# bitsauce/Carla-ppo

Measured on NVIDIA H100. Metric: VAE frames/sec @ batch 4096, higher is better.
Workload: dtype f32

## Files before the change

carla_ppo_b200/csrc/tc_tapgemm.cu:

```cuda
#include "tapgemm.cuh"
#include "tc_common.cuh"

namespace cpb {

namespace {

using namespace tc;

template <int BN, int PASSES>
struct TcCfg {
    static constexpr int B_TILE_BYTES = BN * TBK * 4;
    static constexpr int B_IMAGES = PASSES == 3 ? 2 : 1;
    static constexpr int STAGE_BYTES = A_TILE_BYTES + B_IMAGES * B_TILE_BYTES;
    static constexpr int STAGES = 200 * 1024 / STAGE_BYTES;
    static constexpr int SMEM_BYTES = STAGES * STAGE_BYTES + 1024;
};
constexpr int CHUNK_KB = 4;

constexpr int kConsumerWarps = 8;
constexpr int kLoaderWarp0 = 8;
constexpr int kLoaderWarps = 4;
constexpr int kLoaderThreads = kLoaderWarps * 32;
constexpr int kTcThreads = 384;

int g_tc_cluster = 1;
int g_tc_clusters[2][2] = {{0, 0}, {0, 0}};

__device__ __forceinline__ uint32_t cluster_ctarank() { uint32_t r; asm volatile("mov.u32 %0, %%cluster_ctarank;" : "=r"(r)); return r; }
__device__ __forceinline__ uint32_t cluster_id_x() { uint32_t r; asm volatile("mov.u32 %0, %%clusterid.x;" : "=r"(r)); return r; }
__device__ __forceinline__ uint32_t cluster_count_x() { uint32_t r; asm volatile("mov.u32 %0, %%nclusterid.x;" : "=r"(r)); return r; }
__device__ __forceinline__ void cluster_sync_all() {
    asm volatile("barrier.cluster.arrive.release.aligned;" ::: "memory");
    asm volatile("barrier.cluster.wait.acquire.aligned;" ::: "memory");
}
__device__ __forceinline__ void mbar_expect_tx(uint64_t* bar, uint32_t bytes) {
    asm volatile("{\n\t.reg .b64 st;\n\tmbarrier.arrive.expect_tx.shared::cta.b64 st, [%0], %1;\n\t}" ::"r"(smem_u32(bar)), "r"(bytes) : "memory");
}
__device__ __forceinline__ void bulk_g2s(uint32_t dst, const void* src, uint32_t bytes, uint64_t* bar, uint16_t mask, bool multicast) {
    if (multicast)
        asm volatile("cp.async.bulk.shared::cluster.global.mbarrier::complete_tx::bytes.multicast::cluster [%0], [%1], %2, [%3], %4;"
                     ::"r"(dst), "l"(src), "r"(bytes), "r"(smem_u32(bar)), "h"(mask) : "memory");
    else
        asm volatile("cp.async.bulk.shared::cluster.global.mbarrier::complete_tx::bytes [%0], [%1], %2, [%3];"
                     ::"r"(dst), "l"(src), "r"(bytes), "r"(smem_u32(bar)) : "memory");
}

template <int BN, int PASSES, bool KSPLIT>
__global__ void __maxnreg__(168)
tc_tapgemm_kernel(const __grid_constant__ TapGemmParams p, const int mgroups, const int total_w) {
    static_assert(PASSES == 3 || PASSES == 1, "3xTF32 or a single TF32 pass");
    using Cfg = TcCfg<BN, PASSES>;
    constexpr int STAGES = Cfg::STAGES;
    constexpr int B_TILE_BYTES = Cfg::B_TILE_BYTES;
    constexpr int STAGE_BYTES = Cfg::STAGE_BYTES;

    extern __shared__ uint8_t smem_raw[];
    __shared__ uint64_t full_bar[STAGES];
    __shared__ uint64_t empty_bar[STAGES];

    const int tid = threadIdx.x;
    const int warp = __shfl_sync(0xffffffffu, tid >> 5, 0), lane = tid & 31;
    const int ntn = p.N / BN;
    const int CS = (int)p.cluster;
    const int rank = CS > 1 ? (int)cluster_ctarank() : 0;
    const int cl_id = CS > 1 ? (int)cluster_id_x() : (int)blockIdx.x;
    const int cl_n = CS > 1 ? (int)cluster_count_x() : (int)gridDim.x;
    const uint16_t cl_mask = (uint16_t)((1u << CS) - 1u);
    const uint32_t smem_base = (smem_u32(smem_raw) + 1023u) & ~1023u;

    if (tid == 0) {
#pragma unroll
        for (int s = 0; s < STAGES; ++s) { mbar_init(&full_bar[s], kLoaderThreads + 1); mbar_init(&empty_bar[s], (uint32_t)(kConsumerWarps * CS)); }
        asm volatile("fence.mbarrier_init.release.cluster;" ::: "memory");
    }
    __syncthreads();
    if (CS > 1) cluster_sync_all();

    auto st_z = [&](int st) { return st / (ntn * mgroups); };
    auto st_y = [&](int st) { return st % ntn; };
    auto st_m0 = [&](int st) { return (long long)(((st / ntn) % mgroups) * CS + rank) * TBM; };
    const int kb_per_tap = p.C / TBK;
    const int ksplit = KSPLIT ? p.ksplit : 1;
    auto split_kb = [&](int nkb, int ks) { return (int)((long long)nkb * ks / ksplit); };

    if (warp >= kLoaderWarp0) {
        const int tl = tid - kLoaderWarp0 * 32;
        const int a_chunk = tl & 7;
        const uint32_t a_soff0 = (uint32_t)((tl >> 6) * 1024 + ((tl >> 3) & 7) * 128 + ((a_chunk ^ ((tl >> 3) & 7)) << 4));
        constexpr int RPT = TBM / (kLoaderThreads / 8);

        int wA = cl_id, stA = 0, tapA = 0, cA = 0;
        int kbLeftA = 0;
        int ntapsA = 0;
        int offA = 0;
        uint32_t tapbitA = 1u;
        const TapClass* clsA = &p.cls[0];
        uint32_t a_base[RPT];
        uint32_t a_taps[RPT];
        auto setup_rows = [&]() {
            stA = KSPLIT ? wA / ksplit : wA;
            const int ksA = wA - stA * ksplit;
            clsA = &p.cls[st_z(stA)];
            ntapsA = clsA->ntaps;
            const int Wo = clsA->Wo, HoWo = clsA->Ho * Wo;
            const long long M = (long long)p.batch * HoWo;
            const uint32_t wo_magic = row_magic(Wo);
            long long m = st_m0(stA) + (tl >> 3);
            int n = (int)(m / HoWo);
            int rem = (int)(m - (long long)n * HoWo);
#pragma unroll
            for (int i = 0; i < RPT; ++i) {
                const bool ok = m < M;
                const int oy = row_of(rem, wo_magic);
                const int ox = rem - oy * Wo;
                const int iy = oy * p.sstride, ix = ox * p.sstride;
                a_base[i] = (uint32_t)n * (uint32_t)p.src_img + (uint32_t)((iy * p.Ws + ix) * p.src_pitch + a_chunk * 4);
                uint32_t bits = 0xffffffffu;
                if (p.check) {
                    bits = 0u;
                    for (int t = 0; t < ntapsA; ++t)
                        if ((unsigned)(iy + clsA->taps[t].dy) < (unsigned)p.Hs && (unsigned)(ix + clsA->taps[t].dx) < (unsigned)p.Ws) bits |= 1u << t;
                }
                a_taps[i] = ok ? bits : 0u;
                m += 16; rem += 16;
                while (rem >= HoWo) { rem -= HoWo; ++n; }
            }
            if constexpr (KSPLIT) {
                const int nkb = ntapsA * kb_per_tap;
                const int kb0 = split_kb(nkb, ksA);
                kbLeftA = split_kb(nkb, ksA + 1) - kb0;
                tapA = kb0 / kb_per_tap;
                cA = (kb0 - tapA * kb_per_tap) * TBK;
                offA = (int)clsA->taps[tapA].src_off + cA;
                tapbitA = 1u << tapA;
            } else {
                offA = (int)clsA->taps[0].src_off;
                tapbitA = 1u;
            }
        };
        if (wA < total_w) setup_rows();
        auto issue_a = [&](uint32_t stage, uint64_t* full) {
            const uint32_t dst = stage + a_soff0;
#pragma unroll
            for (int i = 0; i < RPT; ++i) {
                const bool v = (a_taps[i] & tapbitA) != 0u;
                const uint32_t off = v ? a_base[i] + (uint32_t)offA : 0u;
                const uint32_t bytes = (v && !(p.debug & 4)) ? 16u : 0u;
                if (p.debug & 2) continue;
                asm volatile("cp.async.cg.shared.global [%0], [%1], 16, %2;" ::"r"(dst + i * 2048), "l"(p.src + off), "r"(bytes) : "memory");
            }
            asm volatile("cp.async.mbarrier.arrive.noinc.shared::cta.b64 [%0];" ::"r"(smem_u32(full)) : "memory");
            cA += TBK; offA += TBK;
            if constexpr (KSPLIT) {
                if (--kbLeftA == 0) {
                    wA += cl_n;
                    if (wA < total_w) setup_rows();
                } else if (cA == p.C) {
                    cA = 0;
                    ++tapA;
                    offA = (int)clsA->taps[tapA].src_off;
                    tapbitA <<= 1;
                }
            } else if (cA == p.C) {
                cA = 0;
                if (++tapA == ntapsA) {
                    tapA = 0;
                    wA += cl_n;
                    if (wA < total_w) setup_rows();
                } else {
                    offA = (int)clsA->taps[tapA].src_off;
                    tapbitA <<= 1;
                }
            }
        };

        constexpr int B_BYTES = Cfg::B_IMAGES * B_TILE_BYTES;
        const uint32_t slice = (uint32_t)(B_BYTES / CS);
        auto issue_b = [&](uint32_t stage, uint64_t* full) {
            if (p.debug & 8) { mbar_arrive(full); return; }
            mbar_expect_tx(full, (uint32_t)B_BYTES);
            const float* wt = p.wk_hi + 2 * clsA->taps[tapA].w_off + ((long long)st_y(stA) * kb_per_tap + cA / TBK) * (2 * BN * TBK);
            bulk_g2s(stage + A_TILE_BYTES + (uint32_t)rank * slice, reinterpret_cast<const char*>(wt) + (size_t)rank * slice,
                     slice, full, cl_mask, CS > 1);
        };

        int sS = 0;
        uint32_t phS = 1;
        while (wA < total_w) {
            mbar_wait(&empty_bar[sS], phS);
            if (tl == 0) issue_b(smem_base + sS * STAGE_BYTES, &full_bar[sS]);
            issue_a(smem_base + sS * STAGE_BYTES, &full_bar[sS]);
            if (++sS == STAGES) { sS = 0; phS ^= 1u; }
        }
    } else {
        constexpr int HALF = BN / 2;
        const int wg = warp >> 2;
        float acc[HALF];
        float dm[HALF], dc[HALF];
#pragma unroll
        for (int i = 0; i < HALF; ++i) { acc[i] = 0.f; dm[i] = 0.f; dc[i] = 0.f; }

        auto epilogue = [&](int st, int ks) {
            const TapClass& cls = p.cls[st_z(st)];
            float* const dst = KSPLIT ? p.dst + (long long)ks * p.kpartial_stride : p.dst;
            const int Wo = cls.Wo, HoWo = cls.Ho * Wo;
            const int col0 = st_y(st) * BN + 2 * (lane & 3);
            const int lcb = p.quad_lcb;
#pragma unroll
            for (int h = 0; h < 2; ++h) {
                const long long m = st_m0(st) + wg * 64 + (warp & 3) * 16 + (lane >> 2) + 8 * h;
                if (m >= (long long)p.batch * HoWo) continue;
                const int n = (int)(m / HoWo);
                const int rem = (int)(m - (long long)n * HoWo);
                const int oy = rem / Wo;
                const int ox = rem - oy * Wo;
                const uint32_t img = (uint32_t)n * (uint32_t)p.dst_img;
                const uint32_t off_plain = img + (uint32_t)(((oy * p.dstride + cls.py) * p.Wd + (ox * p.dstride + cls.px)) * p.dst_pitch);
                constexpr int NG = BN / 8;
                constexpr int GB = NG < 4 ? NG : 4;
#pragma unroll
                for (int j0 = 0; j0 < NG; j0 += GB) {
                    uint32_t offs[GB];
                    int chs[GB];
                    bool oks[GB];
                    float2 mks[GB];
#pragma unroll
                    for (int u = 0; u < GB; ++u) {
                        const int col = col0 + (j0 + u) * 8;
                        oks[u] = true;
                        if (p.quad) {
                            const int c = col >> lcb;
                            chs[u] = col & (p.quad_cb - 1);
                            const int y = oy * 2 + (c >> 1), x = ox * 2 + (c & 1);
                            oks[u] = y < p.Hd && x < p.Wd;
                            offs[u] = img + (uint32_t)((y * p.Wd + x) * p.dst_pitch + chs[u]);
                        } else {
                            chs[u] = col;
                            offs[u] = off_plain + (uint32_t)col;
                        }
                    }
                    if (p.mask) {
#pragma unroll
                        for (int u = 0; u < GB; ++u)
                            mks[u] = oks[u] ? __ldg(reinterpret_cast<const float2*>(p.mask + offs[u])) : make_float2(0.f, 0.f);
                    }
#pragma unroll
                    for (int u = 0; u < GB; ++u) {
                        if (!oks[u]) continue;
                        const int r = 4 * (j0 + u) + 2 * h;
                        float2 o = make_float2(acc[r], acc[r + 1]);
                        if (p.bias) {
                            const float2 b = __ldg(reinterpret_cast<const float2*>(p.bias + chs[u]));
                            o.x += b.x; o.y += b.y;
                        }
                        if (p.relu) { o.x = fmaxf(o.x, 0.f); o.y = fmaxf(o.y, 0.f); }
                        if (p.mask) { o.x = mks[u].x > 0.f ? o.x : 0.f; o.y = mks[u].y > 0.f ? o.y : 0.f; }
                        *reinterpret_cast<float2*>(dst + offs[u]) = o;
                    }
                }
            }
        };

        auto release = [&](int s) {
            if (lane < CS) {
                if (CS > 1) mbar_arrive_cluster(&empty_bar[s], (uint32_t)lane);
                else mbar_arrive(&empty_bar[s]);
            }
        };

        const int r0 = wg * 64 + (warp & 3) * 16 + (lane >> 2);
        const uint32_t a_row = (uint32_t)((r0 >> 3) * 1024 + (r0 & 7) * 128 + (lane & 3) * 4);
        const uint32_t a_swz = (uint32_t)((r0 & 7) << 4);

        int g = 0;
        for (int w = cl_id; w < total_w; w += cl_n) {
            const int st = KSPLIT ? w / ksplit : w, ks = KSPLIT ? w - st * ksplit : 0;
            const int nkb_tile = p.cls[st_z(st)].ntaps * kb_per_tap;
            const int nkb = KSPLIT ? split_kb(nkb_tile, ks + 1) - split_kb(nkb_tile, ks) : nkb_tile;
            for (int kb = 0; kb < nkb; ++kb, ++g) {
                const int s = g % STAGES;
                const uint32_t stage = smem_base + s * STAGE_BYTES;
                mbar_wait(&full_bar[s], (uint32_t)((g / STAGES) & 1));
                uint32_t ahi[TBK / 8][4], alo[TBK / 8][4];
#pragma unroll
                for (int ks = 0; ks < TBK / 8; ++ks)
#pragma unroll
                    for (int h = 0; h < 2; ++h)
#pragma unroll
                        for (int v = 0; v < 2; ++v) {
                            float x;
                            asm volatile("ld.shared.f32 %0, [%1];" : "=f"(x)
                                         : "r"(stage + a_row + v * 1024 + ((uint32_t)((2 * ks + h) << 4) ^ a_swz)));
                            if constexpr (PASSES == 3) {
                                float hi, lo;
                                split_tf32(x, hi, lo);
                                ahi[ks][2 * h + v] = __float_as_uint(hi);
                                alo[ks][2 * h + v] = __float_as_uint(lo);
                            } else {
                                ahi[ks][2 * h + v] = round_tf32(x);
                            }
                        }
#pragma unroll
                for (int ks = 0; ks < TBK / 8; ++ks)
#pragma unroll
                    for (int i = 0; i < 4; ++i) {
                        if constexpr (PASSES == 3) asm volatile("" : "+r"(ahi[ks][i]), "+r"(alo[ks][i]));
                        else asm volatile("" : "+r"(ahi[ks][i]));
                    }
                const uint64_t b_hi = make_desc(stage + A_TILE_BYTES);
                const uint64_t b_lo = make_desc(stage + A_TILE_BYTES + B_TILE_BYTES);
                wgmma_fence();
#pragma unroll
                for (int ks = 0; ks < TBK / 8; ++ks) {
                    const uint64_t adv = (uint64_t)(ks * 2);
                    const uint32_t keep = ((kb % CHUNK_KB) | ks) != 0 ? 1u : 0u;
                    wgmma_tf32_rs<BN>(dm, ahi[ks], b_hi + adv, keep);
                    if constexpr (PASSES == 3) {
                        wgmma_tf32_rs<BN>(dc, ahi[ks], b_lo + adv, keep);
                        wgmma_tf32_rs<BN>(dc, alo[ks], b_hi + adv, 1u);
                    }
                }
                wgmma_commit();
                wgmma_wait<0>();
                fence_regs<HALF>(dm);
                if constexpr (PASSES == 3) fence_regs<HALF>(dc);
                release(s);
                if (kb % CHUNK_KB == CHUNK_KB - 1 || kb == nkb - 1) {
#pragma unroll
                    for (int i = 0; i < HALF; ++i) {
                        acc[i] += dm[i];
                        if constexpr (PASSES == 3) acc[i] += dc[i];
                    }
                }
            }
            epilogue(st, ks);
#pragma unroll
            for (int i = 0; i < HALF; ++i) acc[i] = 0.f;
        }
    }
    __syncthreads();
    if (CS > 1) cluster_sync_all();
}

constexpr int tc_bn_slot(int BN) { return BN == 64 ? 1 : 0; }
constexpr int tc_passes_slot(int PASSES) { return PASSES == 1 ? 1 : 0; }

template <int BN, int PASSES, bool KSPLIT>
int32_t tc_launch_t(const TapGemmParams& p, int mgroups, int total_w, unsigned grid, cudaStream_t stream) {
    cudaLaunchConfig_t cfg;
    memset(&cfg, 0, sizeof(cfg));
    cfg.gridDim = dim3(grid);
    cfg.blockDim = dim3(kTcThreads);
    cfg.dynamicSmemBytes = TcCfg<BN, PASSES>::SMEM_BYTES;
    cfg.stream = stream;
    cudaLaunchAttribute attr;
    attr.id = cudaLaunchAttributeClusterDimension;
    attr.val.clusterDim.x = (unsigned)p.cluster; attr.val.clusterDim.y = 1; attr.val.clusterDim.z = 1;
    cfg.attrs = &attr; cfg.numAttrs = 1;
    CPB_CUDA(cudaLaunchKernelEx(&cfg, tc_tapgemm_kernel<BN, PASSES, KSPLIT>, p, mgroups, total_w));
    CPB_LAUNCHED();
    return CPB_OK;
}

template <int BN, int PASSES>
int32_t tc_launch(const TapGemmParams& p0, cudaStream_t stream) {
    long long max_m = 0;
    for (int c = 0; c < p0.nclass; ++c) {
        long long m = (long long)p0.batch * p0.cls[c].Ho * p0.cls[c].Wo;
        if (m > max_m) max_m = m;
    }
    if (max_m == 0) return CPB_OK;
    TapGemmParams p = p0;
    p.cluster = g_tc_cluster;
    const long long mtiles = (max_m + TBM - 1) / TBM;
    const long long mgroups = (mtiles + p.cluster - 1) / p.cluster;
    const long long total_w = mgroups * (p.N / BN) * p.nclass * p.ksplit;
    const int resident = g_tc_clusters[tc_passes_slot(PASSES)][tc_bn_slot(BN)];
    CPB_REQUIRE(total_w < (1ll << 30) && resident > 0, "tc_tapgemm: bad tile count");
    CPB_REQUIRE(tc_offsets_fit(p.batch, p.src_img) && tc_offsets_fit(p.batch, p.dst_img),
                "tc_tapgemm: tensors too large for 32-bit row offsets");
    for (int c = 0; c < p.nclass; ++c) CPB_REQUIRE(p.cls[c].ntaps <= 32, "tc_tapgemm: more than 32 taps");
    if (p.quad) {
        CPB_REQUIRE((p.quad_cb & (p.quad_cb - 1)) == 0, "tc_tapgemm: quad form needs a power-of-two channel count");
        p.quad_lcb = 0;
        while ((1 << p.quad_lcb) < p.quad_cb) ++p.quad_lcb;
    }
    const unsigned grid = (unsigned)((total_w < resident ? total_w : resident) * p.cluster);
    if (p.ksplit == 1) return tc_launch_t<BN, PASSES, false>(p, (int)mgroups, (int)total_w, grid, stream);
    if constexpr (PASSES == 1) {
        TapGemmParams q = p;
        q.dst = p.kpartial; q.bias = nullptr; q.mask = nullptr; q.relu = 0;
        CPB_TRY((tc_launch_t<BN, PASSES, true>(q, (int)mgroups, (int)total_w, grid, stream)));
        return launch_ksplit_reduce(p, stream);
    } else {
        CPB_REQUIRE(false, "tc_tapgemm: the k-split is built for the single TF32 pass only");
        return CPB_ERR_UNSUPPORTED;
    }
}

template <int BN, int PASSES>
int32_t tc_init_one() {
    using Cfg = TcCfg<BN, PASSES>;
    CPB_CUDA(cudaFuncSetAttribute(tc_tapgemm_kernel<BN, PASSES, false>, cudaFuncAttributeMaxDynamicSharedMemorySize, Cfg::SMEM_BYTES));
    if (g_tc_cluster > 1) CPB_CUDA(cudaFuncSetAttribute(tc_tapgemm_kernel<BN, PASSES, false>, cudaFuncAttributeNonPortableClusterSizeAllowed, 1));
    if constexpr (PASSES == 1) {
        CPB_CUDA(cudaFuncSetAttribute(tc_tapgemm_kernel<BN, PASSES, true>, cudaFuncAttributeMaxDynamicSharedMemorySize, Cfg::SMEM_BYTES));
        if (g_tc_cluster > 1) CPB_CUDA(cudaFuncSetAttribute(tc_tapgemm_kernel<BN, PASSES, true>, cudaFuncAttributeNonPortableClusterSizeAllowed, 1));
    }
    cudaLaunchConfig_t cfg;
    memset(&cfg, 0, sizeof(cfg));
    cfg.gridDim = dim3((unsigned)(g_tc_cluster * 1024));
    cfg.blockDim = dim3(kTcThreads);
    cfg.dynamicSmemBytes = Cfg::SMEM_BYTES;
    cudaLaunchAttribute attr;
    attr.id = cudaLaunchAttributeClusterDimension;
    attr.val.clusterDim.x = (unsigned)g_tc_cluster; attr.val.clusterDim.y = 1; attr.val.clusterDim.z = 1;
    cfg.attrs = &attr; cfg.numAttrs = 1;
    int n = 0;
    CPB_CUDA(cudaOccupancyMaxActiveClusters(&n, tc_tapgemm_kernel<BN, PASSES, false>, &cfg));
    CPB_REQUIRE(n > 0, "tc_tapgemm: no resident cluster of %d CTAs possible", g_tc_cluster);
    g_tc_clusters[tc_passes_slot(PASSES)][tc_bn_slot(BN)] = n;
    return CPB_OK;
}

__global__ void tc_weights_kernel(const float* __restrict__ params, float* __restrict__ dst, const __grid_constant__ TcWeightTable t) {
    long long idx = (long long)blockIdx.x * blockDim.x + threadIdx.x;
    if (idx >= t.total) return;
    int j = 0;
    while (j < t.njobs - 1 && idx >= t.jobs[j].count) { idx -= t.jobs[j].count; ++j; }
    const TcWeightJob& job = t.jobs[j];
    float x;
    int tap, n, c;
    if (job.mode == 0) {
        tap = 0; n = (int)(idx / job.C); c = (int)(idx % job.C);
        x = params[job.src_off + idx];
    } else if (job.mode == 3) {
        tap = 0; n = (int)(idx / job.C); c = (int)(idx % job.C);
        x = params[job.src_off + (long long)c * job.N + n];
    } else if (job.mode == 2) {
        const int w = (job.k + 1) / 2;
        const int cs = (int)(idx % job.cs);
        long long rest = idx / job.cs;
        const int ncol = (int)(rest % (4 * job.cb));
        rest /= (4 * job.cb);
        const int i = (int)(rest % w), jj = (int)(rest / w);
        const int cls = ncol / job.cb, cb = ncol - cls * job.cb;
        const int kh = (cls >> 1) + 2 * jj, kw = (cls & 1) + 2 * i;
        x = (kh < job.k && kw < job.k) ? params[job.src_off + (((long long)kh * job.k + kw) * job.cb + cb) * job.cs + cs] : 0.f;
        tap = jj * w + i; n = ncol; c = cs;
    } else {
        const int run = job.k * job.cb;
        const int cc = (int)(idx % run);
        const long long rest = idx / run;
        const int cs = (int)(rest % job.cs);
        const int kh = (int)(rest / job.cs);
        const int kw = cc / job.cb, cb = cc - kw * job.cb;
        x = params[job.src_off + (((long long)kh * job.k + kw) * job.cb + cb) * job.cs + cs];
        tap = kh; n = cs; c = cc;
    }
    const int BN = tc_bn(job.N);
    const int nn = n % BN, cc = c % TBK;
    const long long block = ((long long)tap * (job.N / BN) + n / BN) * (job.C / TBK) + c / TBK;
    const long long at = job.dst_hi + block * (2 * BN * TBK) + (nn >> 3) * 256 + (nn & 7) * 32 + ((((cc >> 2) ^ (nn & 7))) << 2) + (cc & 3);
    const float hi = job.round_nearest ? __uint_as_float(round_tf32(x)) : __uint_as_float(__float_as_uint(x) & 0xffffe000u);
    dst[at] = hi;
    if (!job.round_nearest) dst[at + BN * TBK] = x - hi;
}

}

int32_t tc_tapgemm_init() {
    const char* e = getenv("CPB_TC_CLUSTER");
    g_tc_cluster = e ? atoi(e) : 1;
    CPB_REQUIRE(g_tc_cluster == 1 || g_tc_cluster == 2 || g_tc_cluster == 4 || g_tc_cluster == 8, "CPB_TC_CLUSTER must be 1, 2, 4 or 8");
    CPB_TRY((tc_init_one<32, 3>()));
    CPB_TRY((tc_init_one<64, 3>()));
    CPB_TRY((tc_init_one<32, 1>()));
    CPB_TRY((tc_init_one<64, 1>()));
    return CPB_OK;
}

int tc_tapgemm_pick_ksplit(int K) {
    const int s = (int)cdiv(K / TBK, 320);
    return s < 1 ? 1 : (s > 4 ? 4 : s);
}

bool tc_tapgemm_supported(const TapGemmParams& p) {
    if (p.quad && (p.N != 4 * p.quad_cb || p.nclass != 1)) return false;
    if (p.ksplit < 1 || p.ksplit > kMaxKSplit) return false;
    if (p.ksplit > 1 && (p.nclass != 1 || p.quad || p.cls[0].Ho != 1 || p.cls[0].Wo != 1 || p.dst_pitch != p.N ||
                         p.kpartial == nullptr || p.cls[0].ntaps * (p.C / TBK) < p.ksplit))
        return false;
    return p.ybatch == 1 && p.C % TBK == 0 && p.N % 32 == 0 && p.N > 0 && p.wk_hi != nullptr && p.wk_lo != nullptr;
}

int32_t launch_tc_tapgemm(const TapGemmParams& p, cudaStream_t stream) {
    CPB_REQUIRE(tc_tapgemm_supported(p), "tc_tapgemm: unsupported problem (C=%d, N=%d)", p.C, p.N);
    CPB_REQUIRE(p.passes == 3 || p.passes == 1, "tc_tapgemm: passes must be 3 or 1, got %d", p.passes);
    if (p.passes == 1) return tc_bn(p.N) == 64 ? tc_launch<64, 1>(p, stream) : tc_launch<32, 1>(p, stream);
    return tc_bn(p.N) == 64 ? tc_launch<64, 3>(p, stream) : tc_launch<32, 3>(p, stream);
}

int32_t launch_tc_weights(const float* params, float* dst, const TcWeightTable& table, cudaStream_t stream) {
    if (table.total == 0) return CPB_OK;
    tc_weights_kernel<<<cdiv(table.total, 256), 256, 0, stream>>>(params, dst, table);
    CPB_LAUNCHED();
    return CPB_OK;
}

}
```

Measured before the change: 74000.

## Move tapgemm epilogue to dedicated warps via shared-memory handoff with register reallocation

```diff
diff --git a/carla_ppo_b200/csrc/tc_tapgemm.cu b/carla_ppo_b200/csrc/tc_tapgemm.cu
--- a/carla_ppo_b200/csrc/tc_tapgemm.cu
+++ b/carla_ppo_b200/csrc/tc_tapgemm.cu
@@ -12,8 +12,9 @@
     static constexpr int B_TILE_BYTES = BN * TBK * 4;
     static constexpr int B_IMAGES = PASSES == 3 ? 2 : 1;
     static constexpr int STAGE_BYTES = A_TILE_BYTES + B_IMAGES * B_TILE_BYTES;
-    static constexpr int STAGES = 200 * 1024 / STAGE_BYTES;
-    static constexpr int SMEM_BYTES = STAGES * STAGE_BYTES + 1024;
+    static constexpr int OUT_BYTES = TBM * BN * 4;
+    static constexpr int STAGES = (224 * 1024 - OUT_BYTES) / STAGE_BYTES;
+    static constexpr int SMEM_BYTES = STAGES * STAGE_BYTES + OUT_BYTES + 1024;
 };
 constexpr int CHUNK_KB = 4;
 
@@ -21,7 +22,13 @@
 constexpr int kLoaderWarp0 = 8;
 constexpr int kLoaderWarps = 4;
 constexpr int kLoaderThreads = kLoaderWarps * 32;
-constexpr int kTcThreads = 384;
+constexpr int kEpilogueWarp0 = 12;
+constexpr int kEpilogueWarps = 4;
+constexpr int kEpilogueThreads = kEpilogueWarps * 32;
+constexpr int kTcThreads = 512;
+constexpr int kLaunchRegs = 128, kConsumerRegs = 168, kSideRegs = 80;
+template <int R> __device__ __forceinline__ void reg_grow() { asm volatile("setmaxnreg.inc.sync.aligned.u32 %0;" ::"n"(R)); }
+template <int R> __device__ __forceinline__ void reg_shrink() { asm volatile("setmaxnreg.dec.sync.aligned.u32 %0;" ::"n"(R)); }
 
 int g_tc_cluster = 1;
 int g_tc_clusters[2][2] = {{0, 0}, {0, 0}};
@@ -46,7 +53,7 @@
 }
 
 template <int BN, int PASSES, bool KSPLIT>
-__global__ void __maxnreg__(168)
+__global__ void __maxnreg__(kLaunchRegs)
 tc_tapgemm_kernel(const __grid_constant__ TapGemmParams p, const int mgroups, const int total_w) {
     static_assert(PASSES == 3 || PASSES == 1, "3xTF32 or a single TF32 pass");
     using Cfg = TcCfg<BN, PASSES>;
@@ -57,6 +64,8 @@
     extern __shared__ uint8_t smem_raw[];
     __shared__ uint64_t full_bar[STAGES];
     __shared__ uint64_t empty_bar[STAGES];
+    __shared__ uint64_t out_full;
+    __shared__ uint64_t out_empty;
 
     const int tid = threadIdx.x;
     const int warp = __shfl_sync(0xffffffffu, tid >> 5, 0), lane = tid & 31;
@@ -67,10 +76,13 @@
     const int cl_n = CS > 1 ? (int)cluster_count_x() : (int)gridDim.x;
     const uint16_t cl_mask = (uint16_t)((1u << CS) - 1u);
     const uint32_t smem_base = (smem_u32(smem_raw) + 1023u) & ~1023u;
+    const uint32_t out_base = smem_base + STAGES * STAGE_BYTES;
 
     if (tid == 0) {
 #pragma unroll
         for (int s = 0; s < STAGES; ++s) { mbar_init(&full_bar[s], kLoaderThreads + 1); mbar_init(&empty_bar[s], (uint32_t)(kConsumerWarps * CS)); }
+        mbar_init(&out_full, kConsumerWarps);
+        mbar_init(&out_empty, kEpilogueWarps);
         asm volatile("fence.mbarrier_init.release.cluster;" ::: "memory");
     }
     __syncthreads();
@@ -83,11 +95,114 @@
     const int ksplit = KSPLIT ? p.ksplit : 1;
     auto split_kb = [&](int nkb, int ks) { return (int)((long long)nkb * ks / ksplit); };
 
-    if (warp >= kLoaderWarp0) {
+    if (warp >= kEpilogueWarp0) {
+        reg_shrink<kSideRegs>();
+        constexpr int CPR = BN / 4;
+        constexpr int RPP = kEpilogueThreads / CPR;
+        constexpr int NR = TBM / RPP;
+        constexpr uint32_t SKIP = 0xffffffffu;
+        const int et = tid - kEpilogueWarp0 * 32;
+        const int ec = et % CPR, er = et / CPR;
+        const uint32_t o_src = out_base + (uint32_t)(er * (BN * 4) + ((ec ^ ((er & 3) << 1)) << 4));
+        uint32_t phO = 0;
+        for (int w = cl_id; w < total_w && !(p.debug & 16); w += cl_n) {
+            const int st = KSPLIT ? w / ksplit : w, ks = KSPLIT ? w - st * ksplit : 0;
+            const TapClass& cls = p.cls[st_z(st)];
+            float* const dst = KSPLIT ? p.dst + (long long)ks * p.kpartial_stride : p.dst;
+            const int Wo = cls.Wo, HoWo = cls.Ho * Wo;
+            const uint32_t M = (uint32_t)p.batch * (uint32_t)HoWo;
+            const uint32_t wo_magic = row_magic(Wo);
+            const int col = st_y(st) * BN + ec * 4;
+            int ch = col, qy = 0, qx = 0;
+            if (p.quad) {
+                const int c = col >> p.quad_lcb;
+                ch = col & (p.quad_cb - 1);
+                qy = c >> 1; qx = c & 1;
+            }
+            const uint32_t m0 = (uint32_t)st_m0(st) + (uint32_t)er;
+            const int n0 = (int)(m0 / (uint32_t)HoWo);
+            const int rem0 = (int)(m0 - (uint32_t)n0 * (uint32_t)HoWo);
+            uint32_t m = m0;
+            int n = n0, rem = rem0;
+            auto next_off = [&]() {
+                const int oy = row_of(rem, wo_magic);
+                const int ox = rem - oy * Wo;
+                const uint32_t img = (uint32_t)n * (uint32_t)p.dst_img;
+                bool ok = m < M;
+                uint32_t off;
+                if (p.quad) {
+                    const int y = oy * 2 + qy, x = ox * 2 + qx;
+                    ok = ok && y < p.Hd && x < p.Wd;
+                    off = img + (uint32_t)((y * p.Wd + x) * p.dst_pitch + ch);
+                } else {
+                    off = img + (uint32_t)(((oy * p.dstride + cls.py) * p.Wd + (ox * p.dstride + cls.px)) * p.dst_pitch + col);
+                }
+                m += RPP; rem += RPP;
+                while (rem >= HoWo) { rem -= HoWo; ++n; }
+                return ok ? off : SKIP;
+            };
+            uint32_t keep[NR / 8];
+            if (p.mask) {
+#pragma unroll 1
+                for (int b = 0; b < NR / 8; ++b) {
+                    uint32_t offs[8];
+                    float4 mk[8];
+#pragma unroll
+                    for (int u = 0; u < 8; ++u) offs[u] = next_off();
+#pragma unroll
+                    for (int u = 0; u < 8; ++u)
+                        mk[u] = offs[u] != SKIP ? __ldg(reinterpret_cast<const float4*>(p.mask + offs[u])) : make_float4(0.f, 0.f, 0.f, 0.f);
+                    uint32_t bits = 0u;
+#pragma unroll
+                    for (int u = 0; u < 8; ++u)
+                        bits |= ((mk[u].x > 0.f ? 1u : 0u) | (mk[u].y > 0.f ? 2u : 0u) | (mk[u].z > 0.f ? 4u : 0u) | (mk[u].w > 0.f ? 8u : 0u)) << (4 * u);
+#pragma unroll
+                    for (int q = 0; q < NR / 8 - 1; ++q) keep[q] = keep[q + 1];
+                    keep[NR / 8 - 1] = bits;
+                }
+                m = m0; n = n0; rem = rem0;
+            }
+            float4 bias = make_float4(0.f, 0.f, 0.f, 0.f);
+            if (p.bias) bias = __ldg(reinterpret_cast<const float4*>(p.bias + ch));
+
+            mbar_wait(&out_full, phO);
+            phO ^= 1u;
+#pragma unroll 1
+            for (int b = 0; b < NR / 8; ++b) {
+                uint32_t offs[8];
+                float4 sums[8];
+#pragma unroll
+                for (int u = 0; u < 8; ++u)
+                    asm volatile("ld.shared.v4.f32 {%0, %1, %2, %3}, [%4];" : "=f"(sums[u].x), "=f"(sums[u].y), "=f"(sums[u].z), "=f"(sums[u].w)
+                                 : "r"(o_src + (uint32_t)((8 * b + u) * RPP * BN * 4)));
+#pragma unroll
+                for (int u = 0; u < 8; ++u) offs[u] = next_off();
+                const uint32_t bits = p.mask ? keep[0] : 0u;
+#pragma unroll
+                for (int q = 0; q < NR / 8 - 1; ++q) keep[q] = keep[q + 1];
+#pragma unroll
+                for (int u = 0; u < 8; ++u) {
+                    if (offs[u] == SKIP) continue;
+                    float4 o = sums[u];
+                    if (p.bias) { o.x += bias.x; o.y += bias.y; o.z += bias.z; o.w += bias.w; }
+                    if (p.relu) { o.x = fmaxf(o.x, 0.f); o.y = fmaxf(o.y, 0.f); o.z = fmaxf(o.z, 0.f); o.w = fmaxf(o.w, 0.f); }
+                    if (p.mask) {
+                        const uint32_t k = bits >> (4 * u);
+                        o.x = (k & 1u) ? o.x : 0.f; o.y = (k & 2u) ? o.y : 0.f; o.z = (k & 4u) ? o.z : 0.f; o.w = (k & 8u) ? o.w : 0.f;
+                    }
+                    *reinterpret_cast<float4*>(dst + offs[u]) = o;
+                }
+            }
+            __syncwarp();
+            if (lane == 0) mbar_arrive(&out_empty);
+        }
+    } else if (warp >= kLoaderWarp0) {
+        reg_shrink<kSideRegs>();
         const int tl = tid - kLoaderWarp0 * 32;
         const int a_chunk = tl & 7;
         const uint32_t a_soff0 = (uint32_t)((tl >> 6) * 1024 + ((tl >> 3) & 7) * 128 + ((a_chunk ^ ((tl >> 3) & 7)) << 4));
-        constexpr int RPT = TBM / (kLoaderThreads / 8);
+        constexpr int RPP = kLoaderThreads / 8;
+        constexpr int RPT = TBM / RPP;
 
         int wA = cl_id, stA = 0, tapA = 0, cA = 0;
         int kbLeftA = 0;
@@ -108,22 +223,29 @@
             long long m = st_m0(stA) + (tl >> 3);
             int n = (int)(m / HoWo);
             int rem = (int)(m - (long long)n * HoWo);
+            int iy[RPT], ix[RPT];
 #pragma unroll
             for (int i = 0; i < RPT; ++i) {
-                const bool ok = m < M;
                 const int oy = row_of(rem, wo_magic);
                 const int ox = rem - oy * Wo;
-                const int iy = oy * p.sstride, ix = ox * p.sstride;
-                a_base[i] = (uint32_t)n * (uint32_t)p.src_img + (uint32_t)((iy * p.Ws + ix) * p.src_pitch + a_chunk * 4);
-                uint32_t bits = 0xffffffffu;
-                if (p.check) {
-                    bits = 0u;
-                    for (int t = 0; t < ntapsA; ++t)
-                        if ((unsigned)(iy + clsA->taps[t].dy) < (unsigned)p.Hs && (unsigned)(ix + clsA->taps[t].dx) < (unsigned)p.Ws) bits |= 1u << t;
-                }
-                a_taps[i] = ok ? bits : 0u;
-                m += 16; rem += 16;
+                iy[i] = oy * p.sstride; ix[i] = ox * p.sstride;
+                a_base[i] = (uint32_t)n * (uint32_t)p.src_img + (uint32_t)((iy[i] * p.Ws + ix[i]) * p.src_pitch + a_chunk * 4);
+                a_taps[i] = m < M ? 0xffffffffu : 0u;
+                m += RPP; rem += RPP;
                 while (rem >= HoWo) { rem -= HoWo; ++n; }
+            }
+            if (p.check) {
+                uint32_t in[RPT];
+#pragma unroll
+                for (int i = 0; i < RPT; ++i) in[i] = 0u;
+                for (int t = 0; t < ntapsA; ++t) {
+                    const int dy = clsA->taps[t].dy, dx = clsA->taps[t].dx;
+#pragma unroll
+                    for (int i = 0; i < RPT; ++i)
+                        if ((unsigned)(iy[i] + dy) < (unsigned)p.Hs && (unsigned)(ix[i] + dx) < (unsigned)p.Ws) in[i] |= 1u << t;
+                }
+#pragma unroll
+                for (int i = 0; i < RPT; ++i) a_taps[i] &= in[i];
             }
             if constexpr (KSPLIT) {
                 const int nkb = ntapsA * kb_per_tap;
@@ -193,6 +315,7 @@
             if (++sS == STAGES) { sS = 0; phS ^= 1u; }
         }
     } else {
+        reg_grow<kConsumerRegs>();
         constexpr int HALF = BN / 2;
         const int wg = warp >> 2;
         float acc[HALF];
@@ -200,67 +323,6 @@
 #pragma unroll
         for (int i = 0; i < HALF; ++i) { acc[i] = 0.f; dm[i] = 0.f; dc[i] = 0.f; }
 
-        auto epilogue = [&](int st, int ks) {
-            const TapClass& cls = p.cls[st_z(st)];
-            float* const dst = KSPLIT ? p.dst + (long long)ks * p.kpartial_stride : p.dst;
-            const int Wo = cls.Wo, HoWo = cls.Ho * Wo;
-            const int col0 = st_y(st) * BN + 2 * (lane & 3);
-            const int lcb = p.quad_lcb;
-#pragma unroll
-            for (int h = 0; h < 2; ++h) {
-                const long long m = st_m0(st) + wg * 64 + (warp & 3) * 16 + (lane >> 2) + 8 * h;
-                if (m >= (long long)p.batch * HoWo) continue;
-                const int n = (int)(m / HoWo);
-                const int rem = (int)(m - (long long)n * HoWo);
-                const int oy = rem / Wo;
-                const int ox = rem - oy * Wo;
-                const uint32_t img = (uint32_t)n * (uint32_t)p.dst_img;
-                const uint32_t off_plain = img + (uint32_t)(((oy * p.dstride + cls.py) * p.Wd + (ox * p.dstride + cls.px)) * p.dst_pitch);
-                constexpr int NG = BN / 8;
-                constexpr int GB = NG < 4 ? NG : 4;
-#pragma unroll
-                for (int j0 = 0; j0 < NG; j0 += GB) {
-                    uint32_t offs[GB];
-                    int chs[GB];
-                    bool oks[GB];
-                    float2 mks[GB];
-#pragma unroll
-                    for (int u = 0; u < GB; ++u) {
-                        const int col = col0 + (j0 + u) * 8;
-                        oks[u] = true;
-                        if (p.quad) {
-                            const int c = col >> lcb;
-                            chs[u] = col & (p.quad_cb - 1);
-                            const int y = oy * 2 + (c >> 1), x = ox * 2 + (c & 1);
-                            oks[u] = y < p.Hd && x < p.Wd;
-                            offs[u] = img + (uint32_t)((y * p.Wd + x) * p.dst_pitch + chs[u]);
-                        } else {
-                            chs[u] = col;
-                            offs[u] = off_plain + (uint32_t)col;
-                        }
-                    }
-                    if (p.mask) {
-#pragma unroll
-                        for (int u = 0; u < GB; ++u)
-                            mks[u] = oks[u] ? __ldg(reinterpret_cast<const float2*>(p.mask + offs[u])) : make_float2(0.f, 0.f);
-                    }
-#pragma unroll
-                    for (int u = 0; u < GB; ++u) {
-                        if (!oks[u]) continue;
-                        const int r = 4 * (j0 + u) + 2 * h;
-                        float2 o = make_float2(acc[r], acc[r + 1]);
-                        if (p.bias) {
-                            const float2 b = __ldg(reinterpret_cast<const float2*>(p.bias + chs[u]));
-                            o.x += b.x; o.y += b.y;
-                        }
-                        if (p.relu) { o.x = fmaxf(o.x, 0.f); o.y = fmaxf(o.y, 0.f); }
-                        if (p.mask) { o.x = mks[u].x > 0.f ? o.x : 0.f; o.y = mks[u].y > 0.f ? o.y : 0.f; }
-                        *reinterpret_cast<float2*>(dst + offs[u]) = o;
-                    }
-                }
-            }
-        };
-
         auto release = [&](int s) {
             if (lane < CS) {
                 if (CS > 1) mbar_arrive_cluster(&empty_bar[s], (uint32_t)lane);
@@ -271,6 +333,21 @@
         const int r0 = wg * 64 + (warp & 3) * 16 + (lane >> 2);
         const uint32_t a_row = (uint32_t)((r0 >> 3) * 1024 + (r0 & 7) * 128 + (lane & 3) * 4);
         const uint32_t a_swz = (uint32_t)((r0 & 7) << 4);
+
+        const uint32_t o_dst = (uint32_t)(r0 * (BN * 4) + ((r0 & 3) << 5) + (lane & 3) * 8);
+        uint32_t phE = 1;
+        auto hand_off = [&]() {
+            mbar_wait(&out_empty, phE);
+            phE ^= 1u;
+#pragma unroll
+            for (int j = 0; j < BN / 8; ++j)
+#pragma unroll
+                for (int h = 0; h < 2; ++h)
+                    asm volatile("st.shared.v2.f32 [%0], {%1, %2};" ::"r"(out_base + (uint32_t)(h * 8 * BN * 4) + (o_dst ^ (uint32_t)(j << 5))),
+                                 "f"(acc[4 * j + 2 * h]), "f"(acc[4 * j + 2 * h + 1]) : "memory");
+            __syncwarp();
+            if (lane == 0) mbar_arrive(&out_full);
+        };
 
         int g = 0;
         for (int w = cl_id; w < total_w; w += cl_n) {
@@ -333,7 +410,7 @@
                     }
                 }
             }
-            epilogue(st, ks);
+            if (!(p.debug & 16)) hand_off();
 #pragma unroll
             for (int i = 0; i < HALF; ++i) acc[i] = 0.f;
         }
@@ -379,6 +456,10 @@
     CPB_REQUIRE(total_w < (1ll << 30) && resident > 0, "tc_tapgemm: bad tile count");
     CPB_REQUIRE(tc_offsets_fit(p.batch, p.src_img) && tc_offsets_fit(p.batch, p.dst_img),
                 "tc_tapgemm: tensors too large for 32-bit row offsets");
+    auto al16 = [](const void* q) { return (reinterpret_cast<uintptr_t>(q) & 15u) == 0; };
+    CPB_REQUIRE(al16(p.dst) && al16(p.mask) && al16(p.bias) && p.dst_pitch % 4 == 0 && p.dst_img % 4 == 0 &&
+                    (p.ksplit == 1 || (al16(p.kpartial) && p.kpartial_stride % 4 == 0)),
+                "tc_tapgemm: destination, mask and bias must be 16-byte aligned");
     for (int c = 0; c < p.nclass; ++c) CPB_REQUIRE(p.cls[c].ntaps <= 32, "tc_tapgemm: more than 32 taps");
     if (p.quad) {
         CPB_REQUIRE((p.quad_cb & (p.quad_cb - 1)) == 0, "tc_tapgemm: quad form needs a power-of-two channel count");
```

Measured after the change: 79720, median of 6. 7.7% higher.
